# bxh1/VIDO-SLAM

Hardware: AMD Instinct MI355X
Metric: frames/sec end-to-end (flow+depth+track+local-BA) at 640x480; BA iters/sec (higher is better)
Workload: dtype f32

## Files before the change

include/vido_c.h:

```cpp
#ifndef VIDO_C_H
#define VIDO_C_H
#include <stdint.h>
#include <stddef.h>
#ifdef __cplusplus
extern "C" {
#endif

#define VIDO_OK              0
#define VIDO_E_INVALID      -1
#define VIDO_E_NO_DEVICE    -2
#define VIDO_E_HIP          -3
#define VIDO_E_CAPACITY     -4
#define VIDO_E_NOMEM        -5

#define VIDO_MAX_LEVELS 16

typedef struct vido_ctx vido_ctx;

typedef struct vido_keypoint { float x, y, size, angle, response; int32_t octave; } vido_keypoint;

typedef struct vido_config {
    int32_t device;
    int32_t width, height;
    int32_t max_batch;
// ... 175 lines not shown

int vido_wino3x3_supported(int cin, int cout, int h, int w);
int vido_wino3x3_fills_chip(int n, int cout, int h, int w, int min_wgs);
long long vido_wino3x3_packed_floats(int cin, int cout);
int vido_wino3x3_pack(const float* w, int cin, int cout, float* u_packed);
int vido_wino3x3_bias_act(vido_ctx* ctx, const float* x, const float* u_packed, const float* bias, float* y, int n, int cin, int cout, int h, int w, float slope);
int vido_wino3x3_form(int n, int cin, int cout, int h, int w);
int vido_fc_h_splitk(int rows, int k, int outs);
int vido_fc_h(vido_ctx* ctx, const float* x, const void* w_packed, const float* bias, float* part, float* y, int rows, int k, int outs, float slope);
int vido_conv3x3_h_supported(int n, int cin, int cout, int h, int w);
int vido_conv3x3_h_workgroups(int n, int cout, int h, int w);
int vido_conv3x3_h_bias_act(vido_ctx* ctx, const float* x, const void* w_packed, const float* bias, float* y, int n, int cin, int cout, int h, int w, float slope);
long long vido_wino3x3_packed_floats_form(int cin, int cout, int form);
int vido_wino3x3_pack_form(const float* w, int cin, int cout, int form, float* u_packed);
int vido_wino3x3_bias_act_form(vido_ctx* ctx, const float* x, const float* u_packed, const float* bias, float* y, int n, int cin, int cout, int h, int w, float slope, int form);
int vido_gconv3x3_supported(int H, int W, int cpg_in, int cpg_out);
int64_t vido_gconv3x3_packed_size(int groups, int cpg_in, int cpg_out);
int vido_gconv3x3_bias_act(vido_ctx* ctx, const float* x, const float* in_bias, const float* w_packed, const float* bias, float* y, int groups, int cpg_in, int cpg_out, int H, int W, float slope);
int vido_gconv3x3_s2_supported(int H, int W, int cpg_in, int cpg_out);
int vido_gconv3x3_s2_bias_act(vido_ctx* ctx, const float* x, const float* w_packed, const float* bias, float* y, int groups, int cpg_in, int cpg_out, int H, int W, float slope);
int vido_lfn_reg_front(vido_ctx* ctx, const float* im1, const float* im2, const float* flow, const float* mean, float scale, int B, int C, int H, int W, float* out, int out_channels);
int vido_lfn_reg_tail(vido_ctx* ctx, const float* dist, const float* flow, const float* wx, const float* bx, const float* wy, const float* by, int B, int K, int H, int W, float* out);
int vido_roi_align(vido_ctx* ctx, const float* feat, int B, int C, int H, int W, const float* rois, int n_rois,
                   float spatial_scale, int pooled_h, int pooled_w, int sampling_ratio, float* out, int on_device);
int vido_nms(vido_ctx* ctx, const float* boxes_xyxy, const float* scores, int n, float thresh, int32_t* keep_out,
             int32_t* n_keep, int on_device);
int vido_nms_grouped(vido_ctx* ctx, const float* boxes_xyxy, const float* scores, const int32_t* groups, int n, float thresh,
                     int32_t* keep_out, int32_t* n_keep, int on_device);
int vido_nms_segments(vido_ctx* ctx, const float* boxes_xyxy, const int32_t* groups, const int32_t* seg_off, const int32_t* seg_n, int n_seg, int max_n, int total,
                      float thresh, int32_t* keep_out, int32_t* n_keep);
// ... 88 lines not shown
```

vido-slam_amd/csrc/convsmall.hip:

```cpp
#include "common.hpp"

namespace {
template <int K>
__global__ __launch_bounds__(256) void k_conv_kxk_c2(const float* __restrict__ x, const float* __restrict__ w, const float* __restrict__ bias, const float* __restrict__ res,
                                                     float* __restrict__ y, int Cin, int H, int W)
{
    constexpr int R = K / 2, TS = 16 + K - 1, CC = 8, NT = CC * TS * TS, NL = (NT + 255) / 256, NW = (CC * K * K * 2 + 255) / 256;
    __shared__ float tile[NT];
    __shared__ __attribute__((aligned(8))) float wl[NW * 256];
    const int tid = threadIdx.x, tx = tid & 15, ty = tid >> 4, bx = blockIdx.x * 16, by = blockIdx.y * 16;
    const size_t HW = (size_t)H * W;
    int toff[NL]; bool tin[NL]; int tch[NL];
#pragma unroll
    for (int j = 0; j < NL; j++) {
        const int i = min(tid + 256 * j, NT - 1), c = i / (TS * TS), r = i - c * (TS * TS), yy = r / TS, xx = r - yy * TS, gy = by + yy - R, gx = bx + xx - R;
        tch[j] = c; tin[j] = tid + 256 * j < NT && gy >= 0 && gy < H && gx >= 0 && gx < W;
        toff[j] = min(max(gy, 0), H - 1) * W + min(max(gx, 0), W - 1);
    }
    float tv[NL], wv[NW];
    auto fetch = [&](int c0) {
#pragma unroll
        for (int j = 0; j < NL; j++) { const int c = min(c0 + tch[j], Cin - 1); tv[j] = x[(size_t)c * HW + toff[j]]; }
#pragma unroll
        for (int j = 0; j < NW; j++) {
// ... 17 lines not shown
            const float2* wc = (const float2*)wl + c * K * K;
#pragma unroll
            for (int dy = 0; dy < K; dy++)
#pragma unroll
                for (int dx = 0; dx < K; dx++) {
                    const float v = tc[dy * TS + dx];
                    const float2 ww = wc[dy * K + dx];
                    acc0 = fmaf(v, ww.x, acc0); acc1 = fmaf(v, ww.y, acc1);
                }
        }
    }
    const int gy = by + ty, gx = bx + tx;
    if (gy < H && gx < W) {
        const size_t o = (size_t)gy * W + gx;
        y[o] = acc0 + (res ? res[o] : 0.f); y[HW + o] = acc1 + (res ? res[HW + o] : 0.f);
    }
}

typedef float f32x16s __attribute__((ext_vector_type(16)));
template <int CB, bool RES>
__global__ __launch_bounds__(256) void k_conv1x1_skinny(const float* __restrict__ x, const float* __restrict__ wp, const float* __restrict__ bias, const float* __restrict__ res,
                                                        float* __restrict__ y, int Cin, int Cout, long long HW, float slope, unsigned xbytes, unsigned wbytes)
{
    const int lane = threadIdx.x & 63, wv = __builtin_amdgcn_readfirstlane(threadIdx.x >> 6);
    const long long p0 = ((long long)blockIdx.x * 4 + wv) * 32;
    if (p0 >= HW) return;
    const long long p = min(p0 + (lane & 31), HW - 1);
    const int nkp = Cin >> 1;
    f32x16s acc[CB];
#pragma unroll
// ... 40 lines not shown
}
}

extern "C" {

int vido_conv_kxk_c2(vido_ctx* ctx, const float* x, const float* w, const float* bias, const float* residual, float* y, int cin, int k, int h, int wd)
{
    if (!ctx) return VIDO_E_INVALID;
    if (!x || !w || !y || x == y || cin < 1 || h < 1 || wd < 1 || (k != 3 && k != 5 && k != 7)) return vido_set_error(ctx, VIDO_E_INVALID, "conv_kxk_c2: bad arguments (k = %d)", k);
    HIP_TRY(ctx, hipSetDevice(ctx->device));
    hipStream_t st = ctx->has_ext_stream ? ctx->ext_stream : ctx->stream;
    const dim3 grid((wd + 15) / 16, (h + 15) / 16), blk(256);
    if (k == 7) hipLaunchKernelGGL(k_conv_kxk_c2<7>, grid, blk, 0, st, x, w, bias, residual, y, cin, h, wd);
    else if (k == 5) hipLaunchKernelGGL(k_conv_kxk_c2<5>, grid, blk, 0, st, x, w, bias, residual, y, cin, h, wd);
    else hipLaunchKernelGGL(k_conv_kxk_c2<3>, grid, blk, 0, st, x, w, bias, residual, y, cin, h, wd);
    HIP_TRY(ctx, hipGetLastError());
    return VIDO_OK;
}

int vido_conv1x1_skinny(vido_ctx* ctx, const float* x, const float* w_packed, const float* bias, const float* residual, float* y, int cin, int cout, long long hw, float slope)
{
    if (!ctx) return VIDO_E_INVALID;
    if (!x || !w_packed || !y || x == y || cin < 2 || (cin & 1) || cin > 256 || cout < 1 || cout > 256 || hw < 1 || slope < 0.f || slope > 1.f || 4ll * cin * hw >= (1ll << 32))
        return vido_set_error(ctx, VIDO_E_INVALID, "conv1x1_skinny: no kernel for %d -> %d channels", cin, cout);
    HIP_TRY(ctx, hipSetDevice(ctx->device));
    hipStream_t st = ctx->has_ext_stream ? ctx->ext_stream : ctx->stream;
    const dim3 grid((unsigned)((hw + 127) / 128)), blk(256);
    const int cbn = (cout + 31) / 32;
    const unsigned xb = (unsigned)(4ll * cin * hw), wb = (unsigned)(4ll * cbn * 32 * cin);
#define SK_LAUNCH(CBV) { if (residual) hipLaunchKernelGGL((k_conv1x1_skinny<CBV, true>), grid, blk, 0, st, x, w_packed, bias, residual, y, cin, cout, hw, slope, xb, wb); \
// ... 12 lines not shown
```

vido-slam_amd/csrc/wino.hip:

```cpp
#include "common.hpp"

namespace {
typedef float f32x16 __attribute__((ext_vector_type(16)));
typedef float f32x4 __attribute__((ext_vector_type(4)));
typedef float f32x2 __attribute__((ext_vector_type(2)));

#define WN_OOB 0x40000000u
#ifndef WN_ABLATE
#define WN_ABLATE 0
#endif
struct WnArgs { const float* x; const float* up; const float* bias; float* y; int N, Cin, Cout, H, W, Ht, Wt, T, nchunk, cgroups, total; float slope; int vec2; unsigned xbytes, ubytes; unsigned long long* prof; };

__device__ __forceinline__ f32x2 pk_add(f32x2 a, f32x2 b) { f32x2 r; asm("v_pk_add_f32 %0, %1, %2" : "=v"(r) : "v"(a), "v"(b)); return r; }
__device__ __forceinline__ f32x2 pk_sub(f32x2 a, f32x2 b) { f32x2 r; asm("v_pk_add_f32 %0, %1, %2 neg_lo:[0,1] neg_hi:[0,1]" : "=v"(r) : "v"(a), "v"(b)); return r; }

template <int CW, int TW, int KC, bool ODD, int KSPL = 0>
__global__ __launch_bounds__(256) void k_wino3x3(WnArgs A)
{
    static_assert(CW * TW == 4 && (KC == 8 || KC == 4), "workgroup = 4 waves");
    static_assert(!KSPL || ((KSPL == 4 || KSPL == 2) && CW == 1 && TW == 4 && KC == 4), "the K-split form is the 1 x 4 form with its four tile blocks re-read as (tile block, channel slice) pairs");
    constexpr int KSL = KSPL ? KSPL : 1, KTB = KSPL ? 4 / KSPL : 1;
    constexpr int KS = KC / 2;
    constexpr int U_BLK = 16 * 64 * KS;
    constexpr int UB = KSPL ? KSL : CW;
    constexpr int U_BUF = UB * U_BLK, V_BUF = 16 * TW * KS * 64, V_P = TW * KS * 64;
    constexpr int NJ = TW * KS / 4;
    constexpr int KSTEP = 4 / TW;
    constexpr int PPB = U_BLK * 4 / 1024;
    static_assert(NJ == 2, "the slices below are written for two pairs per thread");
    extern __shared__ __attribute__((aligned(16))) float wn_lds[];
    float* Ul = wn_lds; float* Vl = wn_lds + 2 * U_BUF;
#ifdef WN_PROF
    unsigned long long tk[4] = {0, 0, 0, 0};
    asm volatile("s_memtime %0" : "=s"(tk[0]));
#endif
    const int tid = threadIdx.x, lane = tid & 63, w = __builtin_amdgcn_readfirstlane(tid >> 6);
    const int per = gridDim.x >> 3, item = (blockIdx.x & 7) * per + (blockIdx.x >> 3);
    if (item >= A.total) return;
    const int tb = item / A.cgroups, cg = item - tb * A.cgroups, tile0 = tb * (KSPL ? KTB * 32 : TW * 32);
    const int hw = A.H * A.W, tpi = A.Ht * A.Wt;

    const int tw_t = w % TW, ks0 = w / TW;
    unsigned voff[16];
    {
        const int gt = tile0 + (KSPL ? (w / KSL) * 32 : tw_t * 32) + (lane & 31), gtc = min(gt, A.T - 1);
        const int n = gtc / tpi, rem = gtc - n * tpi, ty = rem / A.Wt, tx = rem - ty * A.Wt;
        unsigned rowo[4], colo[4];
#pragma unroll
        for (int d = 0; d < 4; d++) {
            const int iy = 2 * ty - 1 + d, ix = 2 * tx - 1 + d;
            rowo[d] = (gt < A.T && iy >= 0 && iy < A.H) ? 4u * (((unsigned)n * (unsigned)A.Cin + (unsigned)(lane >> 5)) * (unsigned)hw + (unsigned)(iy * A.W)) : WN_OOB;
            colo[d] = (ix >= 0 && ix < A.W) ? 4u * (unsigned)ix : WN_OOB;
        }
#pragma unroll
        for (int e = 0; e < 16; e++) voff[e] = rowo[e >> 2] + colo[e & 3];
    }
    const unsigned par_oob = (lane >> 5) ? WN_OOB : 0u;
    f32x2 inp[NJ][8];
    auto load_win = [&](int chunk, int j, int e0, int e1) {
        const int cb = (KSPL ? KSL * chunk + w % KSL : chunk) * KC + 2 * (ks0 + j * KSTEP);
        const bool any = cb < A.Cin;
        const __amdgpu_buffer_rsrc_t xr = __builtin_amdgcn_make_buffer_rsrc((void*)A.x, 0, any ? A.xbytes : 0u, 0x00020000);
        const unsigned so = any ? 4u * (unsigned)cb * (unsigned)hw : 0u;
        const unsigned extra = (ODD && cb == A.Cin - 1) ? par_oob : 0u;
#pragma unroll
        for (int e = e0; e < e1; e++)
            inp[j][e >> 1][e & 1] = __builtin_bit_cast(float, __builtin_amdgcn_raw_buffer_load_b32(xr, ODD ? voff[e] + extra : voff[e], so, 0));
    };
    f32x2 R[NJ][8];
    auto xf_rows = [&](int j) {
        const f32x2* D = inp[j];
#pragma unroll
        for (int h = 0; h < 2; h++) {
            asm("v_pk_add_f32 %0, %1, %2 neg_lo:[0,1] neg_hi:[0,1]" : "=v"(R[j][h]) : "v"(D[h]), "v"(D[4 + h]));
            asm("v_pk_add_f32 %0, %1, %2" : "=v"(R[j][2 + h]) : "v"(D[2 + h]), "v"(D[4 + h]));
            asm("v_pk_add_f32 %0, %1, %2 neg_lo:[0,1] neg_hi:[0,1]" : "=v"(R[j][4 + h]) : "v"(D[4 + h]), "v"(D[2 + h]));
            asm("v_pk_add_f32 %0, %1, %2 neg_lo:[0,1] neg_hi:[0,1]" : "=v"(R[j][6 + h]) : "v"(D[2 + h]), "v"(D[6 + h]));
        }
    };
    f32x2 Vo[NJ][8];
    auto xf_cols = [&](int j) {
#pragma unroll
// ... 138 lines not shown
            f32x2* d = red + (((two * (KSL - 1) + ksl - 1) * 8 + (r >> 1)) * 4) * 64 + lane;
            d[0] = y00; d[64] = y01; d[128] = y10; d[192] = y11;
        }
    }
    if (KSPL) { __syncthreads(); if (ksl || gt >= A.T) return; }
#pragma unroll
    for (int r = 0; r < 16; r += 2) {
        f32x2 y00, y01, y10, y11; inverse(r, y00, y01, y10, y11);
        if (KSPL) {
#pragma unroll
            for (int s = 0; s < KSL - 1; s++) {
                const f32x2* d = red + (((two * (KSL - 1) + s) * 8 + (r >> 1)) * 4) * 64 + lane;
                y00 = pk_add(y00, d[0]); y01 = pk_add(y01, d[64]); y10 = pk_add(y10, d[128]); y11 = pk_add(y11, d[192]);
            }
        }
        const f32x2 s00 = y00 * sl, s01 = y01 * sl, s10 = y10 * sl, s11 = y11 * sl;
        y00.x = fmaxf(y00.x, s00.x); y00.y = fmaxf(y00.y, s00.y); y01.x = fmaxf(y01.x, s01.x); y01.y = fmaxf(y01.y, s01.y);
        y10.x = fmaxf(y10.x, s10.x); y10.y = fmaxf(y10.y, s10.y); y11.x = fmaxf(y11.x, s11.x); y11.y = fmaxf(y11.y, s11.y);
        const int co = cob + 8 * (r >> 2) + (r & 3);
        float* yp = yb + (size_t)co * hw;
        if (full) {
            *(f32x2*)yp = f32x2{y00.x, y01.x}; *(f32x2*)(yp + A.W) = f32x2{y10.x, y11.x};
            *(f32x2*)(yp + hw) = f32x2{y00.y, y01.y}; *(f32x2*)(yp + hw + A.W) = f32x2{y10.y, y11.y};
        } else {
#pragma unroll
            for (int h = 0; h < 2; h++) {
                if (co + h >= A.Cout) continue;
                float* q = yp + (size_t)h * hw;
                const float a00 = h ? y00.y : y00.x, a01 = h ? y01.y : y01.x, a10 = h ? y10.y : y10.x, a11 = h ? y11.y : y11.x;
                if (A.vec2) {
                    *(f32x2*)q = f32x2{a00, a01};
                    if (row1) *(f32x2*)(q + A.W) = f32x2{a10, a11};
                } else {
// ... 99 lines not shown
        attr[ctx->device & 63] = true;
    }
    const bool odd = cin & 1;
    if (form == 1) { if (odd) hipLaunchKernelGGL((k_wino3x3<1, 4, 4, true, 4>), grid, blk, LDSK, st, A); else hipLaunchKernelGGL((k_wino3x3<1, 4, 4, false, 4>), grid, blk, LDSK, st, A); }
    else if (form == 2) { if (odd) hipLaunchKernelGGL((k_wino3x3<1, 4, 4, true, 2>), grid, blk, LDSK2, st, A); else hipLaunchKernelGGL((k_wino3x3<1, 4, 4, false, 2>), grid, blk, LDSK2, st, A); }
    else if (kc == 8) { if (odd) hipLaunchKernelGGL((k_wino3x3<2, 2, 8, true>), grid, blk, LDS8, st, A); else hipLaunchKernelGGL((k_wino3x3<2, 2, 8, false>), grid, blk, LDS8, st, A); }
    else { if (odd) hipLaunchKernelGGL((k_wino3x3<1, 4, 4, true>), grid, blk, LDS4, st, A); else hipLaunchKernelGGL((k_wino3x3<1, 4, 4, false>), grid, blk, LDS4, st, A); }
    HIP_TRY(ctx, hipGetLastError());
    return VIDO_OK;
}
int vido_wino3x3_bias_act(vido_ctx* ctx, const float* x, const float* u_packed, const float* bias, float* y, int n, int cin, int cout, int h, int w, float slope)
{
    return vido_wino3x3_bias_act_form(ctx, x, u_packed, bias, y, n, cin, cout, h, w, slope, 0);
}

}
```

vido-slam_amd/nets/fuse.py:

```python
import os
import torch
import torch.nn as nn
import torch.nn.functional as F


def _fold(conv, bn, eps):
    scale = bn.weight * (bn.running_var + eps).rsqrt()
    w = conv.weight * scale.reshape(-1, 1, 1, 1)
    b = bn.bias - bn.running_mean * scale
    if conv.bias is not None:
        b = b + conv.bias * scale
    return w.detach().contiguous(), b.detach().contiguous()


def _eps(bn):
    return float(getattr(bn, "eps", 0.0))


def fold_batchnorm(net, ops):
    from .maskrcnn import _Bottleneck, _Stem
    from .monodepth2 import _Basic, ResnetEncoder18, DepthDecoder
    n = 0
    for m in net.modules():
        if isinstance(m, _Bottleneck):
# ... 12 lines not shown
            m._w1p = m._w3p = m._wdp = None; m._c1x1_min_tiles = 0
            mode = os.environ.get("VIDO_CONV1X1", "all")
            if not os.environ.get("VIDO_NO_CONV1X1") and hasattr(ops, "conv1x1_bias_act"):
                from .ops import PackedConv1x1
                m._w3p = PackedConv1x1.make(m._w3)
                if mode == "all":
                    if tuple(m.conv1.stride) == (1, 1): m._w1p = PackedConv1x1.make(m._w1)
                    if m.downsample is not None and tuple(m.downsample[0].stride) in ((1, 1), (2, 2)): m._wdp = PackedConv1x1.make(m._wd)
        elif isinstance(m, _Stem):
            m._w1, m._b1 = _fold(m.conv1, m.bn1, _eps(m.bn1)); m._ep = ops.bias_res_act_; n += 1
        elif isinstance(m, _Basic):
            m._w1, m._b1 = _fold(m.conv1, m.bn1, m.bn1.eps); m._w2, m._b2 = _fold(m.conv2, m.bn2, m.bn2.eps); n += 2
            if m.downsample is not None:
                m._wd, m._bd = _fold(m.downsample[0], m.downsample[1], m.downsample[1].eps); n += 1
            m._ep = ops.bias_res_act_
        elif isinstance(m, DepthDecoder):
            m._ops = ops if hasattr(ops, "upcat_reflect") and not os.environ.get("VIDO_NO_DEPTH_FUSED") else None
        elif isinstance(m, ResnetEncoder18):
            e = m.encoder
            w, b = _fold(e.conv1, e.bn1, e.bn1.eps)
            m._w1, m._b1 = w, b; m._ep = ops.bias_res_act_; n += 1
    return n


class Graphed:

    def __init__(self, fn, example_inputs, warmup=2):
        self.fn = fn
        self.static_in = [x.clone() for x in example_inputs]
        side = torch.cuda.Stream()
        side.wait_stream(torch.cuda.current_stream())
        with torch.cuda.stream(side):
            for _ in range(warmup):
                fn(*self.static_in)
        torch.cuda.current_stream().wait_stream(side)
        torch.cuda.synchronize()
# ... 12 lines not shown
```

vido-slam_amd/nets/monodepth2.py:

```python
import torch
import torch.nn as nn
import torch.nn.functional as F


class _Basic(nn.Module):
    def __init__(self, cin, cout, stride):
        super().__init__()
        self.conv1 = nn.Conv2d(cin, cout, 3, stride, 1, bias=False); self.bn1 = nn.BatchNorm2d(cout)
        self.conv2 = nn.Conv2d(cout, cout, 3, 1, 1, bias=False); self.bn2 = nn.BatchNorm2d(cout)
        self.downsample = None
        if stride != 1 or cin != cout:
            self.downsample = nn.Sequential(nn.Conv2d(cin, cout, 1, stride, bias=False), nn.BatchNorm2d(cout))

    _ep = None

    def forward(self, x):
        if self._ep is not None and x.is_cuda:
            ep = self._ep
            y = ep(F.conv2d(x, self._w1, None, self.conv1.stride, 1), self._b1, None, 0.0)
            sc = x if self.downsample is None else ep(F.conv2d(x, self._wd, None, self.downsample[0].stride), self._bd, None, 1.0)
            return ep(F.conv2d(y, self._w2, None, 1, 1), self._b2, sc.contiguous(), 0.0)
        y = F.relu(self.bn1(self.conv1(x)))
        y = self.bn2(self.conv2(y))
        return F.relu(y + (x if self.downsample is None else self.downsample(x)))


class _ResNet18Trunk(nn.Module):
    def __init__(self):
        super().__init__()
        self.conv1 = nn.Conv2d(3, 64, 7, 2, 3, bias=False); self.bn1 = nn.BatchNorm2d(64)
        self.layer1 = nn.Sequential(_Basic(64, 64, 1), _Basic(64, 64, 1))
        self.layer2 = nn.Sequential(_Basic(64, 128, 2), _Basic(128, 128, 1))
        self.layer3 = nn.Sequential(_Basic(128, 256, 2), _Basic(256, 256, 1))
        self.layer4 = nn.Sequential(_Basic(256, 512, 2), _Basic(512, 512, 1))
        self.fc = nn.Linear(512, 1000)

# ... 44 lines not shown
    def __init__(self, num_ch_enc=ResnetEncoder18.num_ch_enc, scales=range(4)):
        super().__init__()
        self.scales = list(scales); mods = []; self.index = {}
        for i in range(4, -1, -1):
            cin = num_ch_enc[-1] if i == 4 else self.num_ch_dec[i + 1]
            self.index[("upconv", i, 0)] = len(mods); mods.append(_ConvBlock(cin, self.num_ch_dec[i]))
            cin = self.num_ch_dec[i] + (num_ch_enc[i - 1] if i > 0 else 0)
            self.index[("upconv", i, 1)] = len(mods); mods.append(_ConvBlock(cin, self.num_ch_dec[i]))
        for s in self.scales:
            self.index[("dispconv", s)] = len(mods); mods.append(_Conv3x3(self.num_ch_dec[s], 1))
        self.decoder = nn.ModuleList(mods)

    _ops = None

    def forward_fused(self, feats):
        ops = self._ops; x = feats[-1]
        for i in range(4, -1, -1):
            b0 = self.decoder[self.index[("upconv", i, 0)]].conv; b1 = self.decoder[self.index[("upconv", i, 1)]].conv
            x = ops.bias_unary_(F.conv2d(b0.pad(x), b0.conv.weight, None), b0.conv.bias, "elu")
            x = ops.upcat_reflect(x, feats[i - 1].contiguous() if i > 0 else None)
            x = ops.bias_unary_(F.conv2d(x, b1.conv.weight, None), b1.conv.bias, "elu")
        d0 = self.decoder[self.index[("dispconv", 0)]]
        return {("disp", 0): ops.bias_unary_(F.conv2d(d0.pad(x), d0.conv.weight, None), d0.conv.bias, "sigmoid")}

    def forward(self, feats):
        if self._ops is not None and feats[-1].is_cuda and feats[-1].shape[0] == 1:
            return self.forward_fused(feats)
        out = {}; x = feats[-1]
        for i in range(4, -1, -1):
            x = self.decoder[self.index[("upconv", i, 0)]](x)
            x = F.interpolate(x, scale_factor=2, mode="nearest")
            if i > 0:
                x = torch.cat([x, feats[i - 1]], 1)
            x = self.decoder[self.index[("upconv", i, 1)]](x)
            if i in self.scales:
                out[("disp", i)] = torch.sigmoid(self.decoder[self.index[("dispconv", i)]](x))
        return out

# ... 27 lines not shown
```

vido-slam_amd/nets/ops.py:

```python
import contextlib
import ctypes as C
import os
import torch

_WINO_MIN_WGS = int(os.environ.get("VIDO_WINO_MIN_WGS", "0"))
_CONV3X3_H_MIN_WGS = 0 if os.environ.get("VIDO_CONV3X3_H") == "0" else int(os.environ.get("VIDO_CONV3X3_H_MIN_WGS", "128"))
_CONVDIRECT_SET = os.environ.get("VIDO_CONVDIRECT_SET", "novalu")


def correlation_torch_reference(first, second, stride):
    a, b = first[:, :, ::stride, ::stride], second[:, :, ::stride, ::stride]
    pad = torch.nn.functional.pad(b, (3, 3, 3, 3))
    H, W = a.shape[2], a.shape[3]
    return torch.stack([(a * pad[:, :, p:p + H, o:o + W]).mean(1) for p in range(7) for o in range(7)], 1)


class HipOps:

    _range_safe = 0

    def __init__(self, ctx):
        self.ctx = ctx

    @property
# ... 282 lines not shown
        if _WINO_MIN_WGS > 0 and not self.ctx.lib.vido_wino3x3_fills_chip(int(x.shape[0]), int(w.shape[0]), int(x.shape[2]), int(x.shape[3]), _WINO_MIN_WGS):
            return None
        if (_CONV3X3_H_MIN_WGS > 0 and x.dtype == torch.float32 and not self._range_safe and self.ctx.lib.vido_conv3x3_h_supported(int(x.shape[0]), int(w.shape[1]), int(w.shape[0]), int(x.shape[2]), int(x.shape[3]))
                and self.ctx.lib.vido_conv3x3_h_workgroups(int(x.shape[0]), int(w.shape[0]), int(x.shape[2]), int(x.shape[3])) >= (1 if int(w.shape[0]) == 64 else _CONV3X3_H_MIN_WGS)):
            key = (w.data_ptr(), w._version, str(x.device))
            if getattr(conv, "_c3h_key", None) != key:
                conv._c3h_w = pack_conv3x3_h(w).to(x.device); conv._c3h_key = key
            return self.conv3x3_h_bias_act(x.contiguous(), conv._c3h_w, b, int(w.shape[0]), slope)
        form = self.wino3x3_form(x.shape[0], w.shape[1], w.shape[0], x.shape[2], x.shape[3])
        key = (w.data_ptr(), w._version, str(x.device))
        if getattr(conv, "_wino_key", None) != key:
            conv._wino_u = {}; conv._wino_key = key
        if form not in conv._wino_u:
            conv._wino_u[form] = pack_wino3x3(w, form).to(x.device)
        return self.wino3x3_bias_act(x.contiguous(), conv._wino_u[form], b, int(w.shape[0]), slope, form)

    def conv3x3_h_bias_act(self, x, w_packed, bias, cout, slope):
        assert x.is_cuda and x.is_contiguous() and x.dtype == torch.float32
        N, cin, H, W = x.shape
        assert w_packed.dtype == torch.int16 and w_packed.numel() == 2 * cout * ((cin + 15) // 16 * 16 * 9 + 1), "conv3x3_h: weight not packed by pack_conv3x3_h for this layer"
        out = torch.empty((N, cout, H, W), device=x.device, dtype=torch.float32)
        self.gconv_flops = getattr(self, "gconv_flops", 0.0) + 2.0 * N * cout * cin * 9 * H * W
        self._adopt_stream()
        self.ctx._check(self.ctx.lib.vido_conv3x3_h_bias_act(self.ctx.h, C.c_void_p(x.data_ptr()), C.c_void_p(w_packed.data_ptr()), C.c_void_p(bias.data_ptr()) if bias is not None else None,
                                                             C.c_void_p(out.data_ptr()), int(N), int(cin), int(cout), int(H), int(W), C.c_float(slope)))
        return out

    def fc_h(self, x, w_packed, bias, outs, slope=1.0):
        assert x.is_cuda and x.is_contiguous() and x.dtype == torch.float32 and x.dim() == 2
        rows, k = int(x.shape[0]), int(x.shape[1])
# ... 463 lines not shown
    return wz.reshape(cop // 32, 32, cin // 2, 2).permute(0, 2, 3, 1).contiguous().reshape(cop // 32, cin // 2, 64)


def pack_gconv3x3(w, groups):
    cout, cpg_in = int(w.shape[0]), int(w.shape[1])
    cpg_out = cout // groups
    if tuple(w.shape[2:]) != (3, 3) or cpg_in % 8 or not (cpg_out % 32 == 0 or cpg_out in (8, 16)):
        return None
    w9 = w.detach().reshape(groups, cpg_out, cpg_in // 8, 8, 9)
    if cpg_out % 32 == 0:
        return w9.reshape(groups, cpg_out // 32, 32, cpg_in // 8, 8, 9).permute(0, 1, 3, 5, 4, 2).contiguous()
    pad = w9.new_zeros((groups, 16, cpg_in // 8, 8, 9)); pad[:, :cpg_out] = w9
    return pad.permute(0, 2, 4, 3, 1).contiguous()


def pack_conv_direct(w):
    import numpy as np
    from ..host import load_library
    lib = load_library()
    lib.vido_conv_direct_packed_floats.restype = C.c_longlong
    cout, cin, kh, kw = (int(v) for v in w.shape)
    wh = np.ascontiguousarray(w.detach().to("cpu", torch.float32).numpy())
    n = int(lib.vido_conv_direct_packed_floats(cin, cout, kh, kw))
    if n <= 0:
        raise RuntimeError("vido_conv_direct_pack: no kernel for %d x %d taps" % (kh, kw))
    out = np.empty(n, np.float32)
    rc = lib.vido_conv_direct_pack(C.c_void_p(wh.ctypes.data), cin, cout, kh, kw, C.c_void_p(out.ctypes.data))
    if rc != 0:
        raise RuntimeError("vido_conv_direct_pack: %d" % rc)
    return torch.from_numpy(out)
# ... 20 lines not shown
```

Baseline: 125.9.

## Fuse monodepth decoder reflect-pad, upsample, concat and ELU into native Winograd convs

Adds a Winograd 3x3 variant that reads reflect-padded, nearest-upsampled and concatenated inputs directly from the two source tensors and applies ELU or a residual add plus ReLU in its epilogue. It also adds a small direct conv kernel for the 16- and 1-channel decoder layers with reflect padding and ELU or sigmoid. The monodepth decoder and the ResNet basic blocks route through these kernels when the layer is small enough. This removes the separate pad, upcat and bias-activation passes and their intermediate tensors, at the cost of more template variants and new border-indexing code paths.

```diff
diff --git a/include/vido_c.h b/include/vido_c.h
--- a/include/vido_c.h
+++ b/include/vido_c.h
@@ -213,6 +213,13 @@
 long long vido_wino3x3_packed_floats_form(int cin, int cout, int form);
 int vido_wino3x3_pack_form(const float* w, int cin, int cout, int form, float* u_packed);
 int vido_wino3x3_bias_act_form(vido_ctx* ctx, const float* x, const float* u_packed, const float* bias, float* y, int n, int cin, int cout, int h, int w, float slope, int form);
+int vido_conv3x3_refl_small_supported(int cin, int cout, int h, int w, int up);
+int vido_conv3x3_refl_small(vido_ctx* ctx, const float* x, const float* w, const float* bias, float* y, int cin, int cout, int h, int w_, int up, int act);
+int vido_wino3x3_md_supported(int c1, int c2, int cout, int h, int w, int up, int mode);
+void vido_wino3x3_md_last(int* out);
+int vido_wino3x3_md_window(int c1, int c2, int h, int w, int up, int ty, int tx, int c, long long* out);
+int vido_wino3x3_md(vido_ctx* ctx, const float* x, const float* x2, const float* u_packed, const float* bias, const float* res, float* y, int n, int c1, int c2, int up, int cout, int h, int w,
+                    float slope, int mode);
 int vido_gconv3x3_supported(int H, int W, int cpg_in, int cpg_out);
 int64_t vido_gconv3x3_packed_size(int groups, int cpg_in, int cpg_out);
 int vido_gconv3x3_bias_act(vido_ctx* ctx, const float* x, const float* in_bias, const float* w_packed, const float* bias, float* y, int groups, int cpg_in, int cpg_out, int H, int W, float slope);
diff --git a/vido-slam_amd/csrc/convsmall.hip b/vido-slam_amd/csrc/convsmall.hip
--- a/vido-slam_amd/csrc/convsmall.hip
+++ b/vido-slam_amd/csrc/convsmall.hip
@@ -55,6 +55,69 @@
     if (gy < H && gx < W) {
         const size_t o = (size_t)gy * W + gx;
         y[o] = acc0 + (res ? res[o] : 0.f); y[HW + o] = acc1 + (res ? res[HW + o] : 0.f);
+    }
+}
+
+template <int CO, int ACT>
+__global__ __launch_bounds__(256) void k_conv3x3_refl_small(const float* __restrict__ x, const float* __restrict__ w, const float* __restrict__ bias, float* __restrict__ y,
+                                                            int Cin, int H, int W, int up)
+{
+    constexpr int TS = 18, CC = 8, NT = CC * TS * TS, NL = (NT + 255) / 256, NWE = CC * 9 * CO, NW = (NWE + 255) / 256;
+    __shared__ float tile[NT];
+    __shared__ __attribute__((aligned(16))) float wl[NW * 256];
+    const int tid = threadIdx.x, tx = tid & 15, ty = tid >> 4, bx = blockIdx.x * 16, by = blockIdx.y * 16;
+    const int ws = W >> up; const size_t HWs = (size_t)(H >> up) * ws, HW = (size_t)H * W;
+    int toff[NL], tch[NL];
+#pragma unroll
+    for (int j = 0; j < NL; j++) {
+        const int i = min(tid + 256 * j, NT - 1), c = i / (TS * TS), r = i - c * (TS * TS), yy = r / TS, xx = r - yy * TS;
+        int gy = by + yy - 1, gx = bx + xx - 1;
+        gy = gy < 0 ? -gy : (gy >= H ? 2 * H - 2 - gy : gy); gx = gx < 0 ? -gx : (gx >= W ? 2 * W - 2 - gx : gx);
+        gy = min(max(gy, 0), H - 1); gx = min(max(gx, 0), W - 1);
+        tch[j] = c; toff[j] = (gy >> up) * ws + (gx >> up);
+    }
+    float tv[NL], wv[NW];
+    auto fetch = [&](int c0) {
+#pragma unroll
+        for (int j = 0; j < NL; j++) { const int c = min(c0 + tch[j], Cin - 1); tv[j] = x[(size_t)c * HWs + toff[j]]; }
+#pragma unroll
+        for (int j = 0; j < NW; j++) {
+            const int i = min(tid + 256 * j, NWE - 1), o = i % CO, t = (i / CO) % 9, c = min(c0 + i / (CO * 9), Cin - 1);
+            wv[j] = w[((size_t)o * Cin + c) * 9 + t];
+        }
+    };
+    float acc[CO];
+#pragma unroll
+    for (int o = 0; o < CO; o++) acc[o] = 0.f;
+    fetch(0);
+    for (int c0 = 0; c0 < Cin; c0 += CC) {
+        __syncthreads();
+#pragma unroll
+        for (int j = 0; j < NL; j++) if (tid + 256 * j < NT) tile[tid + 256 * j] = (c0 + tch[j] < Cin) ? tv[j] : 0.f;
+#pragma unroll
+        for (int j = 0; j < NW; j++) { const int i = tid + 256 * j; if (i < NWE) wl[i] = (c0 + i / (CO * 9) < Cin) ? wv[j] : 0.f; }
+        __syncthreads();
+        if (c0 + CC < Cin) fetch(c0 + CC);
+#pragma unroll 2
+        for (int c = 0; c < CC; c++) {
+            const float* tc = tile + c * TS * TS + ty * TS + tx;
+            float s[CO];
+#pragma unroll
+            for (int t = 0; t < 9; t++) {
+                const float v = tc[(t / 3) * TS + (t % 3)];
+                const float* wc = wl + (c * 9 + t) * CO;
+#pragma unroll
+                for (int o = 0; o < CO; o++) s[o] = t ? fmaf(v, wc[o], s[o]) : v * wc[o];
+            }
+#pragma unroll
+            for (int o = 0; o < CO; o++) acc[o] += s[o];
+        }
+    }
+    const int gy = by + ty, gx = bx + tx;
+    if (gy < H && gx < W) {
+        const size_t p = (size_t)gy * W + gx;
+#pragma unroll
+        for (int o = 0; o < CO; o++) { const float v = acc[o] + (bias ? bias[o] : 0.f); y[(size_t)o * HW + p] = ACT == 1 ? (v > 0.f ? v : expf(v) - 1.f) : 1.f / (1.f + expf(-v)); }
     }
 }
 
@@ -125,6 +188,24 @@
     if (k == 7) hipLaunchKernelGGL(k_conv_kxk_c2<7>, grid, blk, 0, st, x, w, bias, residual, y, cin, h, wd);
     else if (k == 5) hipLaunchKernelGGL(k_conv_kxk_c2<5>, grid, blk, 0, st, x, w, bias, residual, y, cin, h, wd);
     else hipLaunchKernelGGL(k_conv_kxk_c2<3>, grid, blk, 0, st, x, w, bias, residual, y, cin, h, wd);
+    HIP_TRY(ctx, hipGetLastError());
+    return VIDO_OK;
+}
+
+int vido_conv3x3_refl_small_supported(int cin, int cout, int h, int wd, int up)
+{
+    return (cout == 16 || cout == 1) && cin >= 1 && cin <= 64 && h >= 2 && wd >= 2 && (up == 0 || (up == 1 && !((h | wd) & 1))) && (long long)h * wd < (1ll << 28);
+}
+int vido_conv3x3_refl_small(vido_ctx* ctx, const float* x, const float* w, const float* bias, float* y, int cin, int cout, int h, int wd, int up, int act)
+{
+    if (!ctx) return VIDO_E_INVALID;
+    if (!x || !w || !y || x == y || (act != 1 && act != 2) || !vido_conv3x3_refl_small_supported(cin, cout, h, wd, up))
+        return vido_set_error(ctx, VIDO_E_INVALID, "conv3x3_refl_small: no kernel for %d -> %d channels on %d x %d (up %d, act %d)", cin, cout, h, wd, up, act);
+    HIP_TRY(ctx, hipSetDevice(ctx->device));
+    hipStream_t st = ctx->has_ext_stream ? ctx->ext_stream : ctx->stream;
+    const dim3 grid((wd + 15) / 16, (h + 15) / 16), blk(256);
+    if (cout == 16) { if (act == 1) hipLaunchKernelGGL((k_conv3x3_refl_small<16, 1>), grid, blk, 0, st, x, w, bias, y, cin, h, wd, up); else hipLaunchKernelGGL((k_conv3x3_refl_small<16, 2>), grid, blk, 0, st, x, w, bias, y, cin, h, wd, up); }
+    else { if (act == 1) hipLaunchKernelGGL((k_conv3x3_refl_small<1, 1>), grid, blk, 0, st, x, w, bias, y, cin, h, wd, up); else hipLaunchKernelGGL((k_conv3x3_refl_small<1, 2>), grid, blk, 0, st, x, w, bias, y, cin, h, wd, up); }
     HIP_TRY(ctx, hipGetLastError());
     return VIDO_OK;
 }
diff --git a/vido-slam_amd/csrc/wino.hip b/vido-slam_amd/csrc/wino.hip
--- a/vido-slam_amd/csrc/wino.hip
+++ b/vido-slam_amd/csrc/wino.hip
@@ -10,12 +10,15 @@
 #define WN_ABLATE 0
 #endif
 struct WnArgs { const float* x; const float* up; const float* bias; float* y; int N, Cin, Cout, H, W, Ht, Wt, T, nchunk, cgroups, total; float slope; int vec2; unsigned xbytes, ubytes; unsigned long long* prof; };
+struct WnArgsMD : WnArgs { const float* x2; const float* res; int C1, ups, wA, hwA; unsigned x2bytes; };
+
+__host__ __device__ inline int wn_border(int i, int n, bool mirror) { return mirror ? (i > n ? -1 : (i < 0 ? -i : (i >= n ? 2 * n - 2 - i : i))) : ((i >= 0 && i < n) ? i : -1); }
 
 __device__ __forceinline__ f32x2 pk_add(f32x2 a, f32x2 b) { f32x2 r; asm("v_pk_add_f32 %0, %1, %2" : "=v"(r) : "v"(a), "v"(b)); return r; }
 __device__ __forceinline__ f32x2 pk_sub(f32x2 a, f32x2 b) { f32x2 r; asm("v_pk_add_f32 %0, %1, %2 neg_lo:[0,1] neg_hi:[0,1]" : "=v"(r) : "v"(a), "v"(b)); return r; }
 
-template <int CW, int TW, int KC, bool ODD, int KSPL = 0>
-__global__ __launch_bounds__(256) void k_wino3x3(WnArgs A)
+template <int CW, int TW, int KC, bool ODD, int KSPL = 0, int MD = 0>
+__global__ __launch_bounds__(256) void k_wino3x3(std::conditional_t<MD != 0, WnArgsMD, WnArgs> A)
 {
     static_assert(CW * TW == 4 && (KC == 8 || KC == 4), "workgroup = 4 waves");
     static_assert(!KSPL || ((KSPL == 4 || KSPL == 2) && CW == 1 && TW == 4 && KC == 4), "the K-split form is the 1 x 4 form with its four tile blocks re-read as (tile block, channel slice) pairs");
@@ -41,31 +44,60 @@
     const int hw = A.H * A.W, tpi = A.Ht * A.Wt;
 
     const int tw_t = w % TW, ks0 = w / TW;
-    unsigned voff[16];
+    unsigned voff[16], voffb[(MD & 4) ? 16 : 1];
     {
         const int gt = tile0 + (KSPL ? (w / KSL) * 32 : tw_t * 32) + (lane & 31), gtc = min(gt, A.T - 1);
         const int n = gtc / tpi, rem = gtc - n * tpi, ty = rem / A.Wt, tx = rem - ty * A.Wt;
         unsigned rowo[4], colo[4];
-#pragma unroll
-        for (int d = 0; d < 4; d++) {
-            const int iy = 2 * ty - 1 + d, ix = 2 * tx - 1 + d;
-            rowo[d] = (gt < A.T && iy >= 0 && iy < A.H) ? 4u * (((unsigned)n * (unsigned)A.Cin + (unsigned)(lane >> 5)) * (unsigned)hw + (unsigned)(iy * A.W)) : WN_OOB;
-            colo[d] = (ix >= 0 && ix < A.W) ? 4u * (unsigned)ix : WN_OOB;
-        }
-#pragma unroll
-        for (int e = 0; e < 16; e++) voff[e] = rowo[e >> 2] + colo[e & 3];
+        if constexpr (MD == 0) {
+#pragma unroll
+            for (int d = 0; d < 4; d++) {
+                const int iy = 2 * ty - 1 + d, ix = 2 * tx - 1 + d;
+                rowo[d] = (gt < A.T && iy >= 0 && iy < A.H) ? 4u * (((unsigned)n * (unsigned)A.Cin + (unsigned)(lane >> 5)) * (unsigned)hw + (unsigned)(iy * A.W)) : WN_OOB;
+                colo[d] = (ix >= 0 && ix < A.W) ? 4u * (unsigned)ix : WN_OOB;
+            }
+#pragma unroll
+            for (int e = 0; e < 16; e++) voff[e] = rowo[e >> 2] + colo[e & 3];
+        } else {
+            const int c1 = (MD & 4) ? A.C1 : A.Cin, sh = (MD & 4) ? A.ups : 0, wa = (MD & 4) ? A.wA : A.W, hwa = (MD & 4) ? A.hwA : hw;
+            unsigned rowb[4], colb[4];
+#pragma unroll
+            for (int d = 0; d < 4; d++) {
+                const int iy = wn_border(2 * ty - 1 + d, A.H, MD & 1), ix = wn_border(2 * tx - 1 + d, A.W, MD & 1);
+                const bool rok = gt < A.T && iy >= 0, cok = ix >= 0;
+                rowo[d] = rok ? 4u * (((unsigned)n * (unsigned)c1 + (unsigned)(lane >> 5)) * (unsigned)hwa + (unsigned)((iy >> sh) * wa)) : WN_OOB;
+                colo[d] = cok ? 4u * (unsigned)(ix >> sh) : WN_OOB;
+                rowb[d] = rok ? 4u * (((unsigned)n * (unsigned)(A.Cin - c1) + (unsigned)(lane >> 5)) * (unsigned)hw + (unsigned)(iy * A.W)) : WN_OOB;
+                colb[d] = cok ? 4u * (unsigned)ix : WN_OOB;
+            }
+#pragma unroll
+            for (int e = 0; e < 16; e++) voff[e] = rowo[e >> 2] + colo[e & 3];
+            if constexpr (MD & 4) {
+#pragma unroll
+                for (int e = 0; e < 16; e++) voffb[e] = rowb[e >> 2] + colb[e & 3];
+            }
+        }
     }
     const unsigned par_oob = (lane >> 5) ? WN_OOB : 0u;
     f32x2 inp[NJ][8];
     auto load_win = [&](int chunk, int j, int e0, int e1) {
         const int cb = (KSPL ? KSL * chunk + w % KSL : chunk) * KC + 2 * (ks0 + j * KSTEP);
         const bool any = cb < A.Cin;
+        if constexpr (MD & 4) {
+            const bool sb = cb >= A.C1;
+            const __amdgpu_buffer_rsrc_t xr = __builtin_amdgcn_make_buffer_rsrc((void*)(sb ? A.x2 : A.x), 0, any ? (sb ? A.x2bytes : A.xbytes) : 0u, 0x00020000);
+            const unsigned so = any ? (sb ? 4u * (unsigned)(cb - A.C1) * (unsigned)hw : 4u * (unsigned)cb * (unsigned)A.hwA) : 0u;
+#pragma unroll
+            for (int e = e0; e < e1; e++)
+                inp[j][e >> 1][e & 1] = __builtin_bit_cast(float, __builtin_amdgcn_raw_buffer_load_b32(xr, sb ? voffb[e] : voff[e], so, 0));
+        } else {
         const __amdgpu_buffer_rsrc_t xr = __builtin_amdgcn_make_buffer_rsrc((void*)A.x, 0, any ? A.xbytes : 0u, 0x00020000);
         const unsigned so = any ? 4u * (unsigned)cb * (unsigned)hw : 0u;
         const unsigned extra = (ODD && cb == A.Cin - 1) ? par_oob : 0u;
 #pragma unroll
         for (int e = e0; e < e1; e++)
             inp[j][e >> 1][e & 1] = __builtin_bit_cast(float, __builtin_amdgcn_raw_buffer_load_b32(xr, ODD ? voff[e] + extra : voff[e], so, 0));
+        }
     };
     f32x2 R[NJ][8];
     auto xf_rows = [&](int j) {
@@ -234,9 +266,27 @@
                 y00 = pk_add(y00, d[0]); y01 = pk_add(y01, d[64]); y10 = pk_add(y10, d[128]); y11 = pk_add(y11, d[192]);
             }
         }
+        if constexpr (MD & 8) {
+            const int co = cob + 8 * (r >> 2) + (r & 3);
+            const float* rp = A.res + ((yb - A.y) + (size_t)co * hw);
+            float q[2][4] = {{0.f, 0.f, 0.f, 0.f}, {0.f, 0.f, 0.f, 0.f}};
+#pragma unroll
+            for (int h = 0; h < 2; h++) {
+                if (co + h >= A.Cout) continue;
+                const float* p = rp + (size_t)h * hw;
+                q[h][0] = p[0]; if (col1) q[h][1] = p[1];
+                if (row1) { q[h][2] = p[A.W]; if (col1) q[h][3] = p[A.W + 1]; }
+            }
+            y00.x += q[0][0]; y01.x += q[0][1]; y10.x += q[0][2]; y11.x += q[0][3]; y00.y += q[1][0]; y01.y += q[1][1]; y10.y += q[1][2]; y11.y += q[1][3];
+        }
+        if constexpr (MD & 2) {
+            auto elu = [](float v) { return v > 0.f ? v : expf(v) - 1.f; };
+            y00.x = elu(y00.x); y00.y = elu(y00.y); y01.x = elu(y01.x); y01.y = elu(y01.y); y10.x = elu(y10.x); y10.y = elu(y10.y); y11.x = elu(y11.x); y11.y = elu(y11.y);
+        } else {
         const f32x2 s00 = y00 * sl, s01 = y01 * sl, s10 = y10 * sl, s11 = y11 * sl;
         y00.x = fmaxf(y00.x, s00.x); y00.y = fmaxf(y00.y, s00.y); y01.x = fmaxf(y01.x, s01.x); y01.y = fmaxf(y01.y, s01.y);
         y10.x = fmaxf(y10.x, s10.x); y10.y = fmaxf(y10.y, s10.y); y11.x = fmaxf(y11.x, s11.x); y11.y = fmaxf(y11.y, s11.y);
+        }
         const int co = cob + 8 * (r >> 2) + (r & 3);
         float* yp = yb + (size_t)co * hw;
         if (full) {
@@ -366,4 +416,64 @@
     return vido_wino3x3_bias_act_form(ctx, x, u_packed, bias, y, n, cin, cout, h, w, slope, 0);
 }
 
-}
+int vido_wino3x3_md_supported(int c1, int c2, int cout, int h, int w, int up, int mode)
+{
+    if (mode != 1 && mode != 2) return 0;
+    if (c1 < 2 || c2 < 0 || (c1 & 1) || (c2 & 1) || (up != 0 && up != 1)) return 0;
+    if (mode == 2 && (c2 || up)) return 0;
+    if (up && ((h | w) & 1)) return 0;
+    return vido_wino3x3_supported(c1 + c2, cout, h, w);
+}
+
+int vido_wino3x3_md_window(int c1, int c2, int h, int w, int up, int ty, int tx, int c, long long* out)
+{
+    if (!out || c < 0 || c >= c1 + c2 || h < 2 || w < 2 || ty < 0 || tx < 0 || ty >= (h + 1) / 2 || tx >= (w + 1) / 2 || (up && ((h | w) & 1))) return VIDO_E_INVALID;
+    const int sh = up ? 1 : 0, ha = h >> sh, wa = w >> sh;
+    for (int e = 0; e < 16; e++) {
+        const int iy = wn_border(2 * ty - 1 + (e >> 2), h, true), ix = wn_border(2 * tx - 1 + (e & 3), w, true);
+        if (iy < 0 || ix < 0) { out[2 * e] = -1; out[2 * e + 1] = 0; continue; }
+        out[2 * e] = c < c1 ? 0 : 1;
+        out[2 * e + 1] = c < c1 ? ((long long)c * ha + (iy >> sh)) * wa + (ix >> sh) : ((long long)(c - c1) * h + iy) * w + ix;
+    }
+    return VIDO_OK;
+}
+
+static int wn_md_last[4] = {-1, -1, 0, 0};
+void vido_wino3x3_md_last(int* out) { for (int i = 0; i < 4; i++) out[i] = wn_md_last[i]; }
+
+int vido_wino3x3_md(vido_ctx* ctx, const float* x, const float* x2, const float* u_packed, const float* bias, const float* res, float* y, int n, int c1, int c2, int up, int cout, int h, int w,
+                    float slope, int mode)
+{
+    if (!ctx) return VIDO_E_INVALID;
+    const int cin = c1 + c2, form = 1;
+    if (!x || !u_packed || !y || x == y || x2 == y || res == y || n < 1 || !vido_wino3x3_md_supported(c1, c2, cout, h, w, up, mode) || (c2 > 0 && !x2) || (mode == 2 && !res)
+        || ((uintptr_t)u_packed & 15) || (((uintptr_t)x | (uintptr_t)x2 | (uintptr_t)res | (uintptr_t)y) & 3))
+        return vido_set_error(ctx, VIDO_E_INVALID, "wino3x3_md: no kernel for mode %d, %d + %d -> %d channels on %d x %d x %d, up %d (or a pointer is missing / misaligned)", mode, c1, c2, cout, n, h, w, up);
+    HIP_TRY(ctx, hipSetDevice(ctx->device));
+    hipStream_t st = ctx->has_ext_stream ? ctx->ext_stream : ctx->stream;
+    const int kc = 4, ht = (h + 1) / 2, wt = (w + 1) / 2, ha = h >> up, wa = w >> up;
+    const long long T = (long long)n * ht * wt;
+    if (T >= (1ll << 30) || 4ll * n * c1 * ha * wa >= (1ll << 30) || 4ll * n * c2 * h * w >= (1ll << 30) || 4ll * n * cout * h * w >= (1ll << 32))
+        return vido_set_error(ctx, VIDO_E_INVALID, "wino3x3_md: a batch of %d images of %d x %d x %d is past the 1 GB the kernel addresses", n, cin, h, w);
+    const int tb = 32, cgroups = (cout + 31) / 32;
+    const long long nblk_ll = (T + tb - 1) / tb;
+    if (nblk_ll * cgroups >= (1ll << 30)) return vido_set_error(ctx, VIDO_E_INVALID, "wino3x3_md: too many work items");
+    const int nblk = (int)nblk_ll, total = nblk * cgroups;
+    WnArgsMD A{{x, u_packed, bias, y, n, cin, cout, h, w, ht, wt, (int)T, wn_cin_pad(cin, kc) / kc, cgroups, total, slope, (w % 2 == 0 && ((uintptr_t)y & 7) == 0) ? 1 : 0, (unsigned)(4ll * n * c1 * ha * wa),
+                (unsigned)(4ll * vido_wino3x3_packed_floats_form(cin, cout, form)), nullptr}, x2, res, c1, up, wa, ha * wa, (unsigned)(4ll * n * c2 * h * w)};
+    const dim3 grid(8 * ((total + 7) / 8)), blk(256);
+    constexpr size_t LDSK = (size_t)2 * (4 * 16 * 64 * 2 + 16 * 4 * 2 * 64) * 4;
+    constexpr int DEC = 7, RES = 8;
+    static bool attr[64] = {};
+    if (!attr[ctx->device & 63]) {
+        for (const void* f : {(const void*)k_wino3x3<1, 4, 4, false, 4, DEC>, (const void*)k_wino3x3<1, 4, 4, false, 4, RES>}) HIP_TRY(ctx, hipFuncSetAttribute(f, hipFuncAttributeMaxDynamicSharedMemorySize, (int)LDSK));
+        attr[ctx->device & 63] = true;
+    }
+    if (mode == 1) hipLaunchKernelGGL((k_wino3x3<1, 4, 4, false, 4, DEC>), grid, blk, LDSK, st, A);
+    else hipLaunchKernelGGL((k_wino3x3<1, 4, 4, false, 4, RES>), grid, blk, LDSK, st, A);
+    HIP_TRY(ctx, hipGetLastError());
+    wn_md_last[0] = form; wn_md_last[1] = mode; wn_md_last[2] = total; wn_md_last[3] = 4;
+    return VIDO_OK;
+}
+
+}
diff --git a/vido-slam_amd/nets/fuse.py b/vido-slam_amd/nets/fuse.py
--- a/vido-slam_amd/nets/fuse.py
+++ b/vido-slam_amd/nets/fuse.py
@@ -50,12 +50,16 @@
             if m.downsample is not None:
                 m._wd, m._bd = _fold(m.downsample[0], m.downsample[1], m.downsample[1].eps); n += 1
             m._ep = ops.bias_res_act_
+            m._ops = ops if hasattr(ops, "wino3x3_md_conv") else None
         elif isinstance(m, DepthDecoder):
             m._ops = ops if hasattr(ops, "upcat_reflect") and not os.environ.get("VIDO_NO_DEPTH_FUSED") else None
         elif isinstance(m, ResnetEncoder18):
             e = m.encoder
             w, b = _fold(e.conv1, e.bn1, e.bn1.eps)
             m._w1, m._b1 = w, b; m._ep = ops.bias_res_act_; n += 1
+            for li, layer in enumerate((e.layer1, e.layer2, e.layer3, e.layer4)):
+                for bi, blk in enumerate(layer):
+                    blk._tag = "layer%d.%d" % (li + 1, bi)
     return n
 
 
diff --git a/vido-slam_amd/nets/monodepth2.py b/vido-slam_amd/nets/monodepth2.py
--- a/vido-slam_amd/nets/monodepth2.py
+++ b/vido-slam_amd/nets/monodepth2.py
@@ -13,13 +13,21 @@
             self.downsample = nn.Sequential(nn.Conv2d(cin, cout, 1, stride, bias=False), nn.BatchNorm2d(cout))
 
     _ep = None
+    _ops = None
+    _tag = ""
 
     def forward(self, x):
         if self._ep is not None and x.is_cuda:
-            ep = self._ep
-            y = ep(F.conv2d(x, self._w1, None, self.conv1.stride, 1), self._b1, None, 0.0)
+            ep = self._ep; ops = self._ops
+            y = None
+            if ops is not None and tuple(self.conv1.stride) == (1, 1):
+                y = ops.wino3x3_f32_conv(self.conv1, self._w1, self._b1, x, 0.0, tag=self._tag + ".conv1")
+            if y is None:
+                y = ep(F.conv2d(x, self._w1, None, self.conv1.stride, 1), self._b1, None, 0.0)
             sc = x if self.downsample is None else ep(F.conv2d(x, self._wd, None, self.downsample[0].stride), self._bd, None, 1.0)
-            return ep(F.conv2d(y, self._w2, None, 1, 1), self._b2, sc.contiguous(), 0.0)
+            sc = sc.contiguous()
+            out = ops.wino3x3_md_conv(self.conv2, self._w2, self._b2, y, res=sc, slope=0.0, mode=2, tag=self._tag + ".conv2") if ops is not None else None
+            return out if out is not None else ep(F.conv2d(y, self._w2, None, 1, 1), self._b2, sc, 0.0)
         y = F.relu(self.bn1(self.conv1(x)))
         y = self.bn2(self.conv2(y))
         return F.relu(y + (x if self.downsample is None else self.downsample(x)))
@@ -94,14 +102,21 @@
     _ops = None
 
     def forward_fused(self, feats):
-        ops = self._ops; x = feats[-1]
+        ops = self._ops; x = feats[-1]; native = hasattr(ops, "wino3x3_md_conv")
         for i in range(4, -1, -1):
             b0 = self.decoder[self.index[("upconv", i, 0)]].conv; b1 = self.decoder[self.index[("upconv", i, 1)]].conv
-            x = ops.bias_unary_(F.conv2d(b0.pad(x), b0.conv.weight, None), b0.conv.bias, "elu")
-            x = ops.upcat_reflect(x, feats[i - 1].contiguous() if i > 0 else None)
-            x = ops.bias_unary_(F.conv2d(x, b1.conv.weight, None), b1.conv.bias, "elu")
+            y = ops.wino3x3_md_conv(b0.conv, b0.conv.weight, b0.conv.bias, x, tag="upconv_%d_0" % i) if native else None
+            if y is None and native:
+                y = ops.conv3x3_refl_small(b0.conv, x, tag="upconv_%d_0.small" % i)
+            x = y if y is not None else ops.bias_unary_(F.conv2d(b0.pad(x), b0.conv.weight, None), b0.conv.bias, "elu")
+            skip = feats[i - 1].contiguous() if i > 0 else None
+            y = ops.wino3x3_md_conv(b1.conv, b1.conv.weight, b1.conv.bias, x, x2=skip, up=True, tag="upconv_%d_1" % i) if native else None
+            if y is None and native and skip is None:
+                y = ops.conv3x3_refl_small(b1.conv, x, up=True, tag="upconv_%d_1.small" % i)
+            x = y if y is not None else ops.bias_unary_(F.conv2d(ops.upcat_reflect(x, skip), b1.conv.weight, None), b1.conv.bias, "elu")
         d0 = self.decoder[self.index[("dispconv", 0)]]
-        return {("disp", 0): ops.bias_unary_(F.conv2d(d0.pad(x), d0.conv.weight, None), d0.conv.bias, "sigmoid")}
+        y = ops.conv3x3_refl_small(d0.conv, x, act="sigmoid", tag="dispconv_0.small") if native else None
+        return {("disp", 0): y if y is not None else ops.bias_unary_(F.conv2d(d0.pad(x), d0.conv.weight, None), d0.conv.bias, "sigmoid")}
 
     def forward(self, feats):
         if self._ops is not None and feats[-1].is_cuda and feats[-1].shape[0] == 1:
diff --git a/vido-slam_amd/nets/ops.py b/vido-slam_amd/nets/ops.py
--- a/vido-slam_amd/nets/ops.py
+++ b/vido-slam_amd/nets/ops.py
@@ -320,6 +320,75 @@
         if form not in conv._wino_u:
             conv._wino_u[form] = pack_wino3x3(w, form).to(x.device)
         return self.wino3x3_bias_act(x.contiguous(), conv._wino_u[form], b, int(w.shape[0]), slope, form)
+
+    wino_md_log = None
+
+    def wino3x3_md_supported(self, c1, c2, cout, H, W, up, mode):
+        return bool(self.ctx.lib.vido_wino3x3_md_supported(int(c1), int(c2), int(cout), int(H), int(W), int(up), int(mode)))
+
+    def wino3x3_md_last(self):
+        out = (C.c_int * 4)()
+        self.ctx.lib.vido_wino3x3_md_last(out)
+        return tuple(int(v) for v in out)
+
+    def wino3x3_md(self, x, x2, u_packed, bias, res, cout, up, slope, mode):
+        assert x.is_cuda and x.is_contiguous() and x.dtype == torch.float32 and u_packed.is_cuda
+        N, c1, h, w = (int(v) for v in x.shape); H, W = (2 * h, 2 * w) if up else (h, w); c2 = 0
+        if x2 is not None:
+            assert x2.is_cuda and x2.is_contiguous() and x2.dtype == torch.float32 and x2.shape[0] == N and tuple(x2.shape[2:]) == (H, W)
+            c2 = int(x2.shape[1])
+        if res is not None:
+            assert res.is_cuda and res.is_contiguous() and res.dtype == torch.float32 and tuple(res.shape) == (N, cout, H, W)
+        out = torch.empty((N, cout, H, W), device=x.device, dtype=torch.float32)
+        self.gconv_flops = getattr(self, "gconv_flops", 0.0) + 2.0 * N * cout * (c1 + c2) * 9 * H * W
+        self._adopt_stream()
+        p = lambda t: C.c_void_p(t.data_ptr()) if t is not None else None
+        self.ctx._check(self.ctx.lib.vido_wino3x3_md(self.ctx.h, p(x), p(x2), p(u_packed), p(bias), p(res), p(out), N, c1, c2, int(bool(up)), int(cout), H, W, C.c_float(slope), int(mode)))
+        return out
+
+    def wino3x3_md_conv(self, holder, w, b, x, x2=None, res=None, up=False, slope=0.0, mode=1, tag=None):
+        N, c1 = int(x.shape[0]), int(x.shape[1]); c2 = int(x2.shape[1]) if x2 is not None else 0; cout = int(w.shape[0])
+        H, W = (2 * int(x.shape[2]), 2 * int(x.shape[3])) if up else (int(x.shape[2]), int(x.shape[3]))
+        ok = (x.is_cuda and x.dtype == torch.float32 and tuple(w.shape[2:]) == (3, 3) and int(w.shape[1]) == c1 + c2 and self.wino3x3_md_supported(c1, c2, cout, H, W, up, mode)
+              and not self.ctx.lib.vido_wino3x3_fills_chip(N, cout, H, W, 128) and monodepth_native_layer(N, c1 + c2, cout, H, W))
+        if self.wino_md_log is not None:
+            self.wino_md_log.append((tag, bool(ok)))
+        if not ok:
+            return None
+        key = (w.data_ptr(), w._version, str(x.device))
+        if getattr(holder, "_wino_md_key", None) != key:
+            holder._wino_md_u = pack_wino3x3(w, 1).to(x.device); holder._wino_md_key = key
+        return self.wino3x3_md(x.contiguous(), x2, holder._wino_md_u, b, res, cout, up, slope, mode)
+
+    def conv3x3_refl_small(self, conv, x, up=False, act="elu", tag=None):
+        w = conv.weight; cout, cin = int(w.shape[0]), int(w.shape[1])
+        H, W = (2 * int(x.shape[2]), 2 * int(x.shape[3])) if up else (int(x.shape[2]), int(x.shape[3]))
+        ok = (x.is_cuda and x.dtype == torch.float32 and x.shape[0] == 1 and int(x.shape[1]) == cin and tuple(w.shape[2:]) == (3, 3) and w.is_contiguous()
+              and bool(self.ctx.lib.vido_conv3x3_refl_small_supported(cin, cout, H, W, int(bool(up)))))
+        if self.wino_md_log is not None:
+            self.wino_md_log.append((tag, bool(ok)))
+        if not ok:
+            return None
+        x = x.contiguous(); b = conv.bias
+        out = torch.empty((1, cout, H, W), device=x.device, dtype=torch.float32)
+        self.gconv_flops = getattr(self, "gconv_flops", 0.0) + 2.0 * cout * cin * 9 * H * W
+        self._adopt_stream()
+        self.ctx._check(self.ctx.lib.vido_conv3x3_refl_small(self.ctx.h, C.c_void_p(x.data_ptr()), C.c_void_p(w.data_ptr()), C.c_void_p(b.data_ptr()) if b is not None else None,
+                                                             C.c_void_p(out.data_ptr()), cin, cout, H, W, int(bool(up)), 1 if act == "elu" else 2))
+        return out
+
+    def wino3x3_f32_conv(self, holder, w, b, x, slope, tag=None):
+        N, cin, H, W = (int(v) for v in x.shape); cout = int(w.shape[0])
+        ok = (x.is_cuda and x.dtype == torch.float32 and tuple(w.shape[2:]) == (3, 3) and int(w.shape[1]) == cin and self.wino3x3_supported(cin, cout, H, W) and 4 * x.numel() < 1 << 30
+              and 4 * N * cout * H * W < 1 << 30 and not self.ctx.lib.vido_wino3x3_fills_chip(N, cout, H, W, 128) and monodepth_native_layer(N, cin, cout, H, W))
+        if self.wino_md_log is not None:
+            self.wino_md_log.append((tag, bool(ok)))
+        if not ok:
+            return None
+        key = (w.data_ptr(), w._version, str(x.device))
+        if getattr(holder, "_wino_md_key", None) != key:
+            holder._wino_md_u = pack_wino3x3(w, 1).to(x.device); holder._wino_md_key = key
+        return self.wino3x3_bias_act(x.contiguous(), holder._wino_md_u, b, cout, slope, 1)
 
     def conv3x3_h_bias_act(self, x, w_packed, bias, cout, slope):
         assert x.is_cuda and x.is_contiguous() and x.dtype == torch.float32
@@ -813,6 +882,10 @@
     return pad.permute(0, 2, 4, 3, 1).contiguous()
 
 
+def monodepth_native_layer(n, cin, cout, h, w):
+    return cin <= 128
+
+
 def pack_conv_direct(w):
     import numpy as np
     from ..host import load_library
```

New measurement: 127.0, median of 6. No clear change (+0.8%).
